# FelixWaiblinger/gym-pybullet-adrp

Measured on AMD Instinct MI355X. Metric: env-steps/sec (N parallel drones) at 1/2/4/8 MI355X; % HBM roofline, higher is better.
Workload: dtype f64; 1 GPU; HoverAviary Physics.PYB 240/30 Hz (8 sub-steps), 4096 envs x 1 drone per GPU, RPM actions, auto-reset; envs_per_gpu=4096, global_envs=4096, drones_per_env=1, parallelism=env-sharded dp1

## Files before the change

### gym_pybullet_adrp_amd/csrc/adrp_device.h

```cpp
#pragma once

#include <hip/hip_runtime.h>
#include <stdint.h>

namespace adrp {

__device__ __forceinline__ void store_out(float4* p, float4 v) {
#ifdef ADRP_NT_STORES
    typedef float f4v __attribute__((ext_vector_type(4)));
    const f4v w = {v.x, v.y, v.z, v.w};
    __builtin_nontemporal_store(w, reinterpret_cast<f4v*>(p));
#else
    *p = v;
#endif
}

#ifdef ADRP_RACE_TIMING
__device__ unsigned long long g_race_phase[32];
#define RACE_MARK(var) const uint64_t var = __builtin_amdgcn_s_memtime()
#define RACE_SET(var) var = __builtin_amdgcn_s_memtime()
#define RACE_ACC(i, dt) do { atomicAdd(&g_race_phase[i], (unsigned long long)(dt)); \
        atomicMax(&g_race_phase[10 + (i)], (unsigned long long)(dt)); } while (0)
constexpr int kWaveSlots = 16384;
__device__ unsigned long long g_race_wave[kWaveSlots * 8];
// ... 350 lines not shown

__device__ __forceinline__ float fatan2_(float y, float x) {
    const float ax = fabsf(x), ay = fabsf(y);
    const float mx = fmaxf(ax, ay), mn = fminf(ax, ay);
    const float a = mx > 0.0f ? mn * __builtin_amdgcn_rcpf(mx) : 0.0f;
    const float t = a * a;
    float p = 0.0028487828094512224f;
    p = p * t - 0.016064105555415154f;
    p = p * t + 0.04268398508429527f;
    p = p * t - 0.07503638416528702f;
    p = p * t + 0.10640615969896317f;
    p = p * t - 0.1420356035232544f;
    p = p * t + 0.19992607831954956f;
    p = p * t - 0.3333307206630707f;
    p = p * t + 1.0f;
    float r = a * p;
    if (ay > ax) r = 1.57079632679489661923f - r;
    if (x < 0.0f) r = 3.14159265358979323846f - r;
    return copysignf(r, y);
}
__device__ __forceinline__ double fatan2_(double y, double x) { return f64::atan2(y, x); }
__device__ __forceinline__ float fatan2_nc_(float y, float x) { return fatan2_(y, x); }
__device__ __forceinline__ double fatan2_nc_(double y, double x) { return f64::atan2_nc(y, x); }
__device__ __forceinline__ float fasin_(float s) { return fatan2_(s, __builtin_amdgcn_sqrtf((1.0f - s) * (1.0f + s))); }
__device__ __forceinline__ double fasin_(double s) { return f64::asin(s); }
__device__ __forceinline__ float fexp_(float x) { return __builtin_amdgcn_exp2f(x * 1.4426950408889634f); }
__device__ __forceinline__ double fexp_(double x) { return f64::exp(x); }

template <typename Real>
struct ChainK {
    Real k004, c100, nn_min, near1, tiny;
    Real ts[3], tc[4];
};
template <typename Real>
__device__ __forceinline__ ChainK<Real> chain_consts() {
    return ChainK<Real>{Real(0.04), Real(100), Real(1e-300), Real(1e-9), Real(0.03),
                        {Real(-0.0001984126984126984), Real(0.008333333333333333), Real(-0.16666666666666666)},
                        {Real(2.48015873015873e-05), Real(-0.001388888888888889), Real(0.041666666666666664), Real(-0.5)}};
}
__device__ __forceinline__ void pin(double& x) { asm volatile("" : "+v"(x)); }
__device__ __forceinline__ void pin(float&) {}
template <typename Real>
__device__ __forceinline__ void pin_all(ChainK<Real>& k) {
    pin(k.k004); pin(k.c100); pin(k.nn_min); pin(k.near1); pin(k.tiny);
#pragma unroll
    for (int i = 0; i < 3; ++i) pin(k.ts[i]);
#pragma unroll
    for (int i = 0; i < 4; ++i) pin(k.tc[i]);
}
__device__ __forceinline__ float hsqrt_nn_(float x, const ChainK<float>&) { return __builtin_amdgcn_sqrtf(x); }
__device__ __forceinline__ double hsqrt_nn_(double x, const ChainK<double>& k) {
    const double y = __builtin_amdgcn_rsq(__builtin_fmax(x, k.nn_min));
    double g = x * y, h = 0.5 * y;
#pragma unroll
    for (int i = 0; i < 2; ++i) {
        const double r = f64::fma_(-g, h, 0.5);
        g = f64::fma_(g, r, g);
        h = f64::fma_(h, r, h);
    }
    const double d = f64::fma_(-g, g, x);
    return f64::fma_(d, h, g);
}
__device__ __forceinline__ void expmap_sinc_cos(float x, float* sinc, float* c, const ChainK<float>&) {
    expmap_sinc_cos(x, sinc, c);
}
__device__ __forceinline__ void expmap_sinc_cos(double x, double* sinc, double* c, const ChainK<double>& k) {
    const double x2 = x * x;
    const bool tiny = __builtin_fabs(x) <= k.tiny;
    double ps = f64::fma_(k.ts[0], x2, k.ts[1]);
    ps = f64::fma_(ps, x2, k.ts[2]);
    double pc = f64::fma_(k.tc[0], x2, k.tc[1]);
    pc = f64::fma_(pc, x2, k.tc[2]);
    pc = f64::fma_(pc, x2, k.tc[3]);
    if (__builtin_expect(!__all(tiny), 0)) {
        double fs, fc;
        expmap_sinc_cos_full(x, &fs, &fc);
        *sinc = tiny ? f64::fma_(x2, ps, 1.0) : fs;
        *c = tiny ? f64::fma_(x2, pc, 1.0) : fc;
        return;
    }
    *sinc = f64::fma_(x2, ps, 1.0);
    *c = f64::fma_(x2, pc, 1.0);
}
__device__ __forceinline__ float quat_inv_norm(float n2, const ChainK<float>&) { return quat_inv_norm(n2); }
__device__ __forceinline__ double quat_inv_norm(double n2, const ChainK<double>& k) {
    const bool near1 = __builtin_fabs(n2 - 1.0) <= k.near1;
    const double newton = f64::fma_(0.5, 1.0 - n2, 1.0);
    if (__builtin_expect(__all(near1), 1)) return newton;
    const double r = f64::rsq_nc(n2);
    return near1 ? newton : r;
}

__device__ __forceinline__ void clamp100_wv(V3<float>& w, V3<float>& v) {
    w = {__builtin_amdgcn_fmed3f(w.x, -100.0f, 100.0f), __builtin_amdgcn_fmed3f(w.y, -100.0f, 100.0f),
         __builtin_amdgcn_fmed3f(w.z, -100.0f, 100.0f)};
    v = {__builtin_amdgcn_fmed3f(v.x, -100.0f, 100.0f), __builtin_amdgcn_fmed3f(v.y, -100.0f, 100.0f),
         __builtin_amdgcn_fmed3f(v.z, -100.0f, 100.0f)};
}
__device__ __forceinline__ double clamp100_sel(double x) { return x < -100.0 ? -100.0 : (x > 100.0 ? 100.0 : x); }
__device__ __forceinline__ void clamp100_wv(V3<double>& w, V3<double>& v) {
    const bool big = (__builtin_fabs(w.x) > 100.0) | (__builtin_fabs(w.y) > 100.0) | (__builtin_fabs(w.z) > 100.0) |
                     (__builtin_fabs(v.x) > 100.0) | (__builtin_fabs(v.y) > 100.0) | (__builtin_fabs(v.z) > 100.0);
    if (__builtin_expect(__any(big), 0)) {
        w = {clamp100_sel(w.x), clamp100_sel(w.y), clamp100_sel(w.z)};
        v = {clamp100_sel(v.x), clamp100_sel(v.y), clamp100_sel(v.z)};
    }
}


template <typename Real>
__device__ __forceinline__ M3<Real> rot(Q4<Real> q) {
    const Real x2 = q.x + q.x, y2 = q.y + q.y, z2 = q.z + q.z;
    const Real xx = q.x * x2, yy = q.y * y2, zz = q.z * z2;
    const Real xy = q.x * y2, xz = q.x * z2, yz = q.y * z2;
    const Real wx = q.w * x2, wy = q.w * y2, wz = q.w * z2;
    return {Real(1) - (yy + zz), xy - wz, xz + wy,
            xy + wz, Real(1) - (xx + zz), yz - wx,
            xz - wy, yz + wx, Real(1) - (xx + yy)};
}
template <typename Real>
__device__ __forceinline__ V3<Real> mul(const M3<Real>& R, V3<Real> v) {
    return {R.a00 * v.x + R.a01 * v.y + R.a02 * v.z,
            R.a10 * v.x + R.a11 * v.y + R.a12 * v.z,
            R.a20 * v.x + R.a21 * v.y + R.a22 * v.z};
}
template <typename Real>
__device__ __forceinline__ V3<Real> mulT(const M3<Real>& R, V3<Real> v) {
    return {R.a00 * v.x + R.a10 * v.y + R.a20 * v.z,
            R.a01 * v.x + R.a11 * v.y + R.a21 * v.z,
            R.a02 * v.x + R.a12 * v.y + R.a22 * v.z};
}
template <typename Real>
__device__ __forceinline__ V3<Real> col2(const M3<Real>& R) {
    return {R.a02, R.a12, R.a22};
}

template <typename Real>
__device__ __forceinline__ V3<Real> euler_xyz(Q4<Real> q) {
    const Real sqx = q.x * q.x, sqy = q.y * q.y, sqz = q.z * q.z, squ = q.w * q.w;
    const Real sarg = Real(-2) * (q.x * q.z - q.w * q.y);
    const Real half_pi = Real(1.57079632679489661923);
    if (sarg <= Real(-0.99999)) return {Real(0), -half_pi, Real(2) * atan2_(q.x, -q.y)};
    if (sarg >= Real(0.99999)) return {Real(0), half_pi, Real(2) * atan2_(-q.x, q.y)};
    return {atan2_(Real(2) * (q.y * q.z + q.w * q.x), squ - sqx - sqy + sqz), asin_(sarg),
            atan2_(Real(2) * (q.x * q.y + q.w * q.z), squ + sqx - sqy - sqz)};
}

template <typename Real>
struct EulerArgs {
    Real sarg, y0, x0, y2, x2;
};
template <typename Real>
__device__ __forceinline__ Real euler_sarg(Q4<Real> q) {
#pragma clang fp contract(on)
    return Real(-2) * (q.x * q.z - q.w * q.y);
}
template <typename Real>
__device__ __forceinline__ EulerArgs<Real> euler_args(Q4<Real> q) {
#pragma clang fp contract(on)
    const Real sqx = q.x * q.x, sqy = q.y * q.y, sqz = q.z * q.z, squ = q.w * q.w;
    const Real sarg = Real(-2) * (q.x * q.z - q.w * q.y);
    const Real y0 = Real(2) * (q.y * q.z + q.w * q.x), x0 = squ - sqx - sqy + sqz;
    const Real y2 = Real(2) * (q.x * q.y + q.w * q.z), x2 = squ + sqx - sqy - sqz;
    return {sarg, y0, x0, y2, x2};
}

// ... 115 lines not shown
```

### gym_pybullet_adrp_amd/csrc/hover_kernel.h

```cpp
#pragma once

#include "adrp_device.h"
#include "dslpid_core.h"

namespace adrp {

enum HoverField {
    HF_POS = 0, HF_QUAT = 3, HF_VEL = 7, HF_OMEGA = 10, HF_LAST_RPM = 13, HF_ANGV = 17,
    HF_LINK_QUAT = 20, HF_NBASE = 24,
    HF_PID = 24, HF_NPID = 9
};
enum HoverInt { HI_STEP = 0, HI_EPISODE = 1, HI_RING_HEAD = 2, HI_N = 3 };

template <typename Real>
struct HoverConst {
    int S, trunc_steps, link_lag, physics;
    Real dt, mass, inv_mass, gravity;
    Real ixx, iyy, izz, inv_ixx, inv_iyy, inv_izz;
    Real kf, km, hover_rpm;
    Real px[4], py[4], pz[4];
    Real gnd_kf, prop_r4, gnd_clip;
    Real drag[3];
    Real dyn_arm;
    Real coll_hh, coll_r, coll_zoff;
// ... 279 lines not shown
    const Real ty = (-f[0] + f[1] + f[2] - f[3]) * a.dyn_arm;
    const V3<Real> rr = b.w;
    const V3<Real> tq = v3(tx, ty, tz) - cross(rr, v3(a.ixx * rr.x, a.iyy * rr.y, a.izz * rr.z));
    const V3<Real> rdd = v3(tq.x * a.inv_ixx, tq.y * a.inv_iyy, tq.z * a.inv_izz);
    b.vel = b.vel + a.dt * (a.inv_mass * force_w);
    b.w = rr + a.dt * rdd;
    b.pos = b.pos + a.dt * b.vel;
    const V3<Real> w = b.w;
    const Real wn = hsqrt_(dot(w, w));
    if (!(wn <= Real(1e-8))) {
        const Real th = wn * a.dt * Real(0.5);
        Real s, c;
        if (th <= Real(0.39269908169872414)) small_sincos(th, &s, &c);
        else sincos_(th, &s, &c);
        const Real k = s * rcp_(wn);
        const Q4<Real> q = b.q;
        b.q = {c * q.x + k * (w.z * q.y - w.y * q.z + w.x * q.w),
               c * q.y + k * (-w.z * q.x + w.x * q.z + w.y * q.w),
               c * q.z + k * (w.y * q.x - w.x * q.y + w.z * q.w),
               c * q.w + k * (-w.x * q.x - w.y * q.y - w.z * q.z)};
    }
    b.angv = mul(R, b.w);
}

template <typename Real>
__device__ __forceinline__ void hover_reset_draw(const HoverReset<Real>& a, uint64_t seed, uint64_t gid, uint32_t tag,
                                                 const HoverConst<Real>& C, Body<Real>& b, int32_t& sc, int32_t& ep) {
    const U4 r0 = draw(seed, gid, uint32_t(ep), tag, 0);
    const U4 r1 = draw(seed, gid, uint32_t(ep), tag, 1);
    const U4 r2 = draw(seed, gid, uint32_t(ep), tag, 2);
    const uint32_t w0[4] = {r0.a, r0.b, r0.c, r0.d}, w1[4] = {r1.a, r1.b, r1.c, r1.d},
                   w2[4] = {r2.a, r2.b, r2.c, r2.d};
    Real p[3], e_[3], v[3], om[3];
#pragma unroll
    for (int k = 0; k < 3; ++k) {
        p[k] = a.init_xyz[k] + a.n_xyz[k] * (Real(2) * u01r<Real>(w0[k]) - Real(1));
        e_[k] = a.init_rpy[k] + a.n_rpy[k] * (Real(2) * u01r<Real>(w1[k]) - Real(1));
        v[k] = a.n_vel[k] * (Real(2) * u01r<Real>(w2[k]) - Real(1));
    }
    om[0] = a.n_om[0] * (Real(2) * u01r<Real>(w0[3]) - Real(1));
    om[1] = a.n_om[1] * (Real(2) * u01r<Real>(w1[3]) - Real(1));
    om[2] = a.n_om[2] * (Real(2) * u01r<Real>(w2[3]) - Real(1));
    b.q = quat_from_euler_fast<Real>(e_[0], e_[1], e_[2]);
    b.pos = v3(p[0], p[1], p[2]);
    b.ql = b.q;
    b.vel = v3(v[0], v[1], v[2]);
    if (C.physics == ADRP_PHYS_DYN) {
        b.w = mulT(rot(b.q), v3(om[0], om[1], om[2]));
        b.angv = v3(om[0], om[1], om[2]);
    } else {
        b.w = v3(om[0], om[1], om[2]);
        b.angv = v3(Real(0), Real(0), Real(0));
    }
#pragma unroll
    for (int i = 0; i < 4; ++i) b.prev_rpm[i] = Real(0);
    sc = 0;
    ep += 1;
}
template <typename Real>
__device__ __forceinline__ void hover_reset_state(const HoverArgs<Real>& args, const HoverConst<Real>& C, int e,
                                                  Body<Real>& b, int32_t& sc, int32_t& ep) {
    hover_reset_draw(*args.r, args.seed, uint64_t(args.env_offset + e), TAG_HOVER_RESET, C, b, sc, ep);
}

template <typename Real>
__device__ __forceinline__ Real euler_roll_u(Q4<Real> q) {
    if (__builtin_expect(__any(fabs_(euler_sarg(q)) >= Real(0.99999)), 0)) return euler_xyz_fast(q).x;
    const EulerArgs<Real> a = euler_args(q);
    return fatan2_(a.y0, a.x0);
}
template <typename Real>
__device__ __forceinline__ Real euler_pitch_u(Q4<Real> q) {
    const Real sarg = euler_sarg(q);
    if (__builtin_expect(__any(fabs_(sarg) >= Real(0.99999)), 0)) return euler_xyz_fast(q).y;
    return fasin_(sarg);
}
template <typename Real>
__device__ __forceinline__ Real euler_yaw_u(Q4<Real> q) {
    if (__builtin_expect(__any(fabs_(euler_sarg(q)) >= Real(0.99999)), 0)) return euler_xyz_fast(q).z;
    const EulerArgs<Real> a = euler_args(q);
    return fatan2_(a.y2, a.x2);
}

template <typename Real>
__device__ __forceinline__ Real euler_axis_u(Q4<Real> q, int ax) {
    const EulerArgs<Real> a = euler_args(q);
    const Real sarg = a.sarg;
    if (__builtin_expect(__any(fabs_(sarg) >= Real(0.99999)), 0)) {
        const V3<Real> r = euler_xyz_fast(q);
        return ax == 0 ? r.x : (ax == 1 ? r.y : r.z);
    }
    const Real y0 = a.y0, x0 = a.x0, y2 = a.y2, x2 = a.x2;
    Real x1;
    if constexpr (sizeof(Real) == 8) x1 = f64::sqrt((1.0 - sarg) * (1.0 + sarg));
    else x1 = __builtin_amdgcn_sqrtf((1.0f - sarg) * (1.0f + sarg));
    const Real yy = ax == 0 ? y0 : (ax == 1 ? sarg : y2), xx = ax == 0 ? x0 : (ax == 1 ? x1 : x2);
    return fatan2_(yy, xx);
}
__device__ __forceinline__ float readlane_r(float v, int l) {
    return __int_as_float(__builtin_amdgcn_readlane(__float_as_int(v), l));
}
__device__ __forceinline__ double readlane_r(double v, int l) {
    return __hiloint2double(__builtin_amdgcn_readlane(__double2hiint(v), l), __builtin_amdgcn_readlane(__double2loint(v), l));
}
template <typename Real>
__device__ __forceinline__ V3<Real> hover_obs12_split(const HoverConst<Real>& a, const Body<Real>& b, float o[12]) {
    const int l = int(threadIdx.x) & 63;
    const Real ang = euler_axis_u(b.q, l < 2 ? l : 2);
    const V3<Real> rpy = v3(readlane_r(ang, 0), readlane_r(ang, 1), readlane_r(ang, 2));
    const V3<Real> w = a.physics == ADRP_PHYS_DYN ? b.angv : b.w;
    o[0] = float(b.pos.x); o[1] = float(b.pos.y); o[2] = float(b.pos.z);
    o[3] = float(rpy.x);   o[4] = float(rpy.y);   o[5] = float(rpy.z);
    o[6] = float(b.vel.x); o[7] = float(b.vel.y); o[8] = float(b.vel.z);
    o[9] = float(w.x);     o[10] = float(w.y);    o[11] = float(w.z);
    return rpy;
}

template <typename Real>
__device__ __forceinline__ V3<Real> hover_obs12(const HoverConst<Real>& a, const Body<Real>& b, float o[12]) {
    const V3<Real> rpy = euler_xyz_fast_u(b.q);
    const V3<Real> w = a.physics == ADRP_PHYS_DYN ? b.angv : b.w;
    o[0] = float(b.pos.x); o[1] = float(b.pos.y); o[2] = float(b.pos.z);
    o[3] = float(rpy.x);   o[4] = float(rpy.y);   o[5] = float(rpy.z);
    o[6] = float(b.vel.x); o[7] = float(b.vel.y); o[8] = float(b.vel.z);
    o[9] = float(w.x);     o[10] = float(w.y);    o[11] = float(w.z);
    return rpy;
}

template <int A, int B>
__device__ __forceinline__ void write_row(float* row, const float o12[12], const float (&ring)[B][A], int head1) {
    if constexpr (A == 4) {
        float4* r4 = reinterpret_cast<float4*>(row);
        r4[0] = make_float4(o12[0], o12[1], o12[2], o12[3]);
        r4[1] = make_float4(o12[4], o12[5], o12[6], o12[7]);
        r4[2] = make_float4(o12[8], o12[9], o12[10], o12[11]);
#pragma unroll
        for (int p = 0; p < B; ++p) {
            int k = p - head1;
            k += k < 0 ? B : 0;
            r4[3 + k] = make_float4(ring[p][0], ring[p][1], ring[p][2], ring[p][3]);
        }
    } else {
#pragma unroll
        for (int k = 0; k < 12; ++k) row[k] = o12[k];
#pragma unroll
        for (int p = 0; p < B; ++p) {
            int k = p - head1;
            k += k < 0 ? B : 0;
#pragma unroll
            for (int j = 0; j < A; ++j) row[12 + k * A + j] = ring[p][j];
        }
    }
}

template <int A>
__device__ __forceinline__ void write_row_generic(float* __restrict__ row, const float o12[12],
                                                  const float* __restrict__ ring, int B, int E, int e, int head1,
                                                  const float act[A], bool act_is_newest) {
#pragma unroll
    for (int k = 0; k < 12; ++k) row[k] = o12[k];
    constexpr int CH = 8;
    int slot = head1;
    for (int k0 = 0; k0 < B; k0 += CH) {
        float v[CH][A];
#pragma unroll
        for (int c = 0; c < CH; ++c) {
// ... 207 lines not shown
        const Real r2 = rpm[i] * rpm[i];
        const Real f = r2 * C.kf;
        sum_f += f;
        const bool pz0 = __builtin_constant_p(C.pz[i]) && C.pz[i] == Real(0);
        const Real fx = f * C.px[i], fy = f * C.py[i], fz = f * C.pz[i];
        P = v3(P.x + fx, P.y + fy, pz0 ? P.z : P.z + fz);
        t2 += (i & 1) ? -r2 : r2;
    }
    const Real tau_z = t2 * C.km;
    ChainK<Real> K = chain_consts<Real>();
    HoverConst<Real> Cp = C;
    if constexpr (sizeof(Real) == 8) {
        pin_all(K);
        pin(Cp.dt); pin(Cp.mass); pin(Cp.gravity); pin(Cp.inv_mass); pin(Cp.ang_max);
        pin(Cp.ixx); pin(Cp.iyy); pin(Cp.izz); pin(Cp.inv_ixx); pin(Cp.inv_iyy); pin(Cp.inv_izz);
        pin(Cp.coll_hh); pin(Cp.coll_r); pin(Cp.coll_zoff);
    }
    Chain<Real> st{};
    {
        const M3<Real> R = rot_fm(b.q);
        const M3<Real> Rs = lag ? rot_fm(b.ql) : R;
        st.wb = mulT(R, b.w);
        st.zc = col2(R);
        st.zs = col2(Rs);
        st.m3 = lag ? mulT(R, st.zs) : v3(Real(0), Real(0), Real(1));
        if constexpr (DRAG) {
            st.R = R;
            st.Rs = Rs;
        }
    }
    st.wn = hsqrt_nn_(dot(b.w, b.w), K);
    st.dti = v3(Cp.dt * Cp.inv_ixx, Cp.dt * Cp.inv_iyy, Cp.dt * Cp.inv_izz);
    bool touched = false;
    auto substep = [&](int s) {
        if constexpr (EXT) touched |= pyb_substep<Real, PH, true>(Cp, b, st, rpm, sum_f, P, tau_z, K, ext(b, st));
        else touched |= pyb_substep<Real, PH>(Cp, b, st, rpm, sum_f, P, tau_z, K, V3<Real>{}, vxy ? vxy + 2 * s : nullptr);
#pragma unroll
        for (int i = 0; i < 4; ++i) b.prev_rpm[i] = rpm[i];
    };
    if constexpr (SC > 0) {
#pragma unroll
        for (int s = 0; s < SC; ++s) substep(s);
    } else {
        for (int s = 0; s < C.S; ++s) substep(s);
    }
    if (wb_out) *wb_out = st.wb;
    else b.w = mul(rot_fm(b.q), st.wb);
    return touched;
}

constexpr int kRowF4 = 18;

template <int A, int B>
__device__ __forceinline__ void stage_row(float4* lds_row, const float o12[12], const float (&ring)[B][A], int head1) {
    lds_row[0] = make_float4(o12[0], o12[1], o12[2], o12[3]);
    lds_row[1] = make_float4(o12[4], o12[5], o12[6], o12[7]);
    lds_row[2] = make_float4(o12[8], o12[9], o12[10], o12[11]);
#pragma unroll
    for (int p = 0; p < B; ++p) {
        int k = p - head1;
        k += k < 0 ? B : 0;
        lds_row[3 + k] = make_float4(ring[p][0], ring[p][1], ring[p][2], ring[p][3]);
    }
}

template <typename Real, int PH, int A, int B, int SC, bool STG = false, int CTL = 0, bool HELP = false, int SYS = 0,
          int FO = 2>
__device__ __forceinline__ void hover_step_body(const HoverArgs<Real>& a, const HoverConst<Real>& C,
                                                const float* pre = nullptr) {
    constexpr int BR = B > 0 ? B : 1;
    constexpr bool DRAG = (PH == ADRP_PHYS_PYB_DRAG || PH == ADRP_PHYS_PYB_GND_DRAG_DW);
    constexpr bool DYN = (PH == ADRP_PHYS_DYN);
    static_assert(!HELP || STG, "the reset helper wave pairs with the staged (all lanes live) kernel");
    __shared__ Real rs_body[HELP ? kResetFields * kStepBlock : 1];
    __shared__ float rs_obs[HELP ? 12 * kStepBlock : 1];
    __shared__ float4 rows[STG ? kStepBlock * kRowF4 : 1];
    constexpr bool ANG = HELP && angle_helpers<Real>();
    __shared__ Real ang_q[ANG ? 4 * kStepBlock : 1];
    __shared__ Real ang_r[ANG ? kStepBlock : 1];
    __shared__ Real ang_p[ANG ? kStepBlock : 1];
    __shared__ float ang_y[ANG ? kStepBlock : 1];
    constexpr int kWaves = HELP ? 1 + help_waves<Real>() : 1;
    constexpr auto cb = [](int w) { return w == 0 ? 0 : (w >= kWaves ? kRowF4 : (kWaves == 2 ? kRowF4 / 2 : 5 * w - 2)); };
    if constexpr (HELP) {
        if (ANG && threadIdx.x >= 2 * kStepBlock) {
            const int tl = threadIdx.x & (kStepBlock - 1), wv = threadIdx.x / kStepBlock;
            __syncthreads();
            const Q4<Real> q = {ang_q[tl], ang_q[kStepBlock + tl], ang_q[2 * kStepBlock + tl], ang_q[3 * kStepBlock + tl]};
            if (wv == 2) ang_p[tl] = euler_pitch_u(q);
            else ang_y[tl] = float(euler_yaw_u(q));
            __syncthreads();
            __syncthreads();
            float4* dst = reinterpret_cast<float4*>(a.obs) + size_t(blockIdx.x) * kStepBlock * kRowF4;
            for (int k = cb(wv); k < cb(wv + 1); ++k) store_out(dst + tl + kStepBlock * k, rows[tl + kStepBlock * k]);
            return;
        }
        if (threadIdx.x >= kStepBlock) {
            const int tl = threadIdx.x - kStepBlock;
            const int he = blockIdx.x * kStepBlock + tl;
            const int E = a.E;
            const float4 av = reinterpret_cast<const float4*>(a.act)[he];
            float rg[BR][4];
#pragma unroll
            for (int p = 0; p < B; ++p) {
                const float4 v = reinterpret_cast<const float4*>(a.ring)[size_t(p) * E + he];
                rg[p][0] = v.x; rg[p][1] = v.y; rg[p][2] = v.z; rg[p][3] = v.w;
            }
            const int32_t head = a.ist[HI_RING_HEAD * E + he];
            int32_t hsc = 0, hep = a.ist[HI_EPISODE * E + he];
            Body<Real> rb;
            hover_reset_state(a, C, he, rb, hsc, hep);
            float o[12];
            hover_obs12(C, rb, o);
            const Real v[kResetFields] = {rb.pos.x, rb.pos.y, rb.pos.z, rb.q.x, rb.q.y, rb.q.z, rb.q.w,
                                          rb.vel.x, rb.vel.y, rb.vel.z, rb.w.x, rb.w.y, rb.w.z,
                                          rb.angv.x, rb.angv.y, rb.angv.z};
#pragma unroll
            for (int k = 0; k < kResetFields; ++k) rs_body[k * kStepBlock + tl] = v[k];
#pragma unroll
            for (int k = 0; k < 12; ++k) rs_obs[k * kStepBlock + tl] = o[k];
            float4* my = rows + tl * kRowF4;
            const int hu = __builtin_amdgcn_readfirstlane(head);
            if (__all(head == hu)) {
                const int h1 = hu + 1 == B ? 0 : hu + 1;
#pragma unroll
                for (int p = 0; p < B; ++p) {
                    const int k = p >= h1 ? p - h1 : p - h1 + B;
                    my[3 + k] = make_float4(rg[p][0], rg[p][1], rg[p][2], rg[p][3]);
                }
                my[3 + B - 1] = av;
            } else {
                const int h1 = head + 1 == B ? 0 : head + 1;
#pragma unroll
                for (int p = 0; p < B; ++p) {
                    int k = p - h1;
                    k += k < 0 ? B : 0;
                    const bool hit = p == head;
                    my[3 + k] = make_float4(hit ? av.x : rg[p][0], hit ? av.y : rg[p][1], hit ? av.z : rg[p][2],
                                            hit ? av.w : rg[p][3]);
                }
            }
            reinterpret_cast<float4*>(a.ring)[size_t(head) * E + he] = av;
            __syncthreads();
            if constexpr (ANG) {
                const Q4<Real> q = {ang_q[tl], ang_q[kStepBlock + tl], ang_q[2 * kStepBlock + tl], ang_q[3 * kStepBlock + tl]};
                ang_r[tl] = euler_roll_u(q);
                __syncthreads();
            }
            __syncthreads();
            float4* dst = reinterpret_cast<float4*>(a.obs) + size_t(blockIdx.x) * kStepBlock * kRowF4;
#pragma unroll
            for (int k = cb(1); k < cb(2); ++k) store_out(dst + tl + kStepBlock * k, rows[tl + kStepBlock * k]);
            return;
        }
    }
    const int E = a.E;
    const bool split = ADRP_PERSIST_SPLIT && !STG && !HELP && E == 1;
    const int e = split ? 0 : int(blockIdx.x) * kStepBlock + int(threadIdx.x);
    const int D = B > 0 ? 12 + B * A : a.D;
    if (e >= E) return;
    RACE_MARK(t0);
    const bool fit = FO == 2 ? field_offsets_fit<Real>(E) : FO == 1;
    const bool lag = C.link_lag && !DYN;
    const BodyOffs<Real> fo = body_offsets<Real>(E, e, lag, DRAG, DYN);
    uint32_t io[HI_N];
    field_run(uint32_t(e) * 4u, uint32_t(E) * 4u, 0, HI_N, io);
    Body<Real> b;
    int32_t sc, ep, head_ld;
    if (fit) {
        load_body_at<Real>(a.f, fo, b, lag, DRAG, DYN);
        sc = field_at(a.ist, io[HI_STEP]); ep = field_at(a.ist, io[HI_EPISODE]); head_ld = field_at(a.ist, io[HI_RING_HEAD]);
        field_form_end();
    } else {
        load_body(a, e, b, lag, DRAG, DYN);
        sc = a.ist[HI_STEP * E + e]; ep = a.ist[HI_EPISODE * E + e]; head_ld = a.ist[HI_RING_HEAD * E + e];
    }
    const int32_t head = head_ld;
    float act[A];
    if constexpr (SYS == 2) {
#pragma unroll
        for (int j = 0; j < A; ++j) act[j] = pre[j];
    } else if constexpr (SYS == 1) {
        uint32_t* sa = const_cast<uint32_t*>(reinterpret_cast<const uint32_t*>(a.act)) + size_t(e) * A;
#pragma unroll
        for (int j = 0; j < A; ++j)
            act[j] = __uint_as_float(__hip_atomic_load(sa + j, __ATOMIC_RELAXED, __HIP_MEMORY_SCOPE_SYSTEM));
    } else if constexpr (A == 4) {
        const float4 v = reinterpret_cast<const float4*>(a.act)[e];
        act[0] = v.x; act[1] = v.y; act[2] = v.z; act[3] = v.w;
    } else {
#pragma unroll
        for (int j = 0; j < A; ++j) act[j] = a.act[e * A + j];
    }
    float ring[BR][A];
#pragma unroll
    for (int p = 0; p < (HELP ? 0 : B); ++p) {
        if constexpr (A == 4) {
            const float4 v = reinterpret_cast<const float4*>(a.ring)[size_t(p) * E + e];
            ring[p][0] = v.x; ring[p][1] = v.y; ring[p][2] = v.z; ring[p][3] = v.w;
        } else {
#pragma unroll
            for (int j = 0; j < A; ++j) ring[p][j] = a.ring[(size_t(p) * E + e) * A + j];
        }
    }
    Real rpm[4];
    if constexpr (CTL != 0) {
        static_assert(A == (CTL == ADRP_ACT_PID ? 3 : CTL == ADRP_ACT_VEL ? 4 : 1), "PID action width");
        Real ctl[HF_NPID];
        uint32_t po[HF_PID + HF_NPID];
        field_run(uint32_t(e) * uint32_t(sizeof(Real)), uint32_t(E) * uint32_t(sizeof(Real)), HF_PID, HF_NPID, po);
        if (fit) {
#pragma unroll
            for (int k = 0; k < HF_NPID; ++k) ctl[k] = field_at(a.f, po[HF_PID + k]);
            field_form_end();
        } else {
#pragma unroll
            for (int k = 0; k < HF_NPID; ++k) ctl[k] = a.f[(HF_PID + k) * E + e];
        }
        dslpid_rpm<Real, CTL>(C, b, act, ctl, rpm);
        if (fit) {
#pragma unroll
            for (int k = 0; k < HF_NPID; ++k) field_last(a.f, po[HF_PID + k]) = ctl[k];
            field_form_end();
        } else {
#pragma unroll
            for (int k = 0; k < HF_NPID; ++k) a.f[(HF_PID + k) * E + e] = ctl[k];
        }
    } else {
#pragma unroll
        for (int i = 0; i < 4; ++i) rpm[i] = C.hover_rpm * Real(rpm_gain(act[A == 1 ? 0 : i]));
    }
    bool touched = false;
// ... 42 lines not shown
    V3<Real> rpy;
    if constexpr (ANG) {
        const int tl = threadIdx.x;
        ang_q[tl] = b.q.x; ang_q[kStepBlock + tl] = b.q.y; ang_q[2 * kStepBlock + tl] = b.q.z;
        ang_q[3 * kStepBlock + tl] = b.q.w;
        __syncthreads();
        hold(b.q.x); hold(b.q.y); hold(b.q.z); hold(b.q.w);
        hold(wbf.x); hold(wbf.y); hold(wbf.z);
        hold(b.pos.x); hold(b.pos.y); hold(b.pos.z);
        if constexpr (LATE_XY) {
#pragma unroll
            for (int k = 0; k < 2 * SC; ++k) hold(vxy[k]);
#pragma unroll
            for (int s = 0; s < SC; ++s) {
                b.pos.x = fmx(C.dt, vxy[2 * s], b.pos.x);
                b.pos.y = fmx(C.dt, vxy[2 * s + 1], b.pos.y);
            }
        }
        hold(b.vel.x); hold(b.vel.y); hold(b.vel.z);
        if constexpr (!DYN) b.w = mul(rot_fm(b.q), wbf);
        const V3<Real> w = C.physics == ADRP_PHYS_DYN ? b.angv : b.w;
        o12[0] = float(b.pos.x); o12[1] = float(b.pos.y); o12[2] = float(b.pos.z);
        o12[6] = float(b.vel.x); o12[7] = float(b.vel.y); o12[8] = float(b.vel.z);
        o12[9] = float(w.x);     o12[10] = float(w.y);    o12[11] = float(w.z);
    } else if (split) {
        rpy = hover_obs12_split(C, b, o12);
    } else {
        rpy = hover_obs12(C, b, o12);
    }
    const Real dx = C.target[0] - b.pos.x, dy = C.target[1] - b.pos.y, dz = C.target[2] - b.pos.z;
    const Real d2 = dx * dx + dy * dy + dz * dz;
    const Real r = Real(2) - d2 * d2;
    a.rew[e] = float(r > Real(0) ? r : Real(0));
    const bool te = d2 < Real(1e-8);
    bool tr = fabs_(b.pos.x) > Real(1.5) || fabs_(b.pos.y) > Real(1.5) || b.pos.z > Real(2.0) || sc >= C.trunc_steps;
    if constexpr (ANG) {
        hold(b.w.x); hold(b.w.y); hold(b.w.z);
#pragma unroll
        for (int k = 0; k < 12; ++k)
            if (k < 3 || k > 5) hold(o12[k]);
        __syncthreads();
        rpy.x = ang_r[threadIdx.x];
        rpy.y = ang_p[threadIdx.x];
        o12[3] = float(rpy.x);
        o12[4] = float(rpy.y);
        o12[5] = ang_y[threadIdx.x];
    }
    tr = tr || fabs_(rpy.x) > Real(0.4) || fabs_(rpy.y) > Real(0.4);
    a.term[e] = te;
    a.trunc[e] = tr;
    sc += C.S;
    const bool done = a.autoreset && (te || tr);
    RACE_MARK(t3);
#ifdef ADRP_RACE_TIMING
    const unsigned long long dmask = __ballot(done);
    uint64_t t4 = 0;
#endif
    if constexpr (STG) {
        static_assert(A == 4 && B == 15, "staged rows: 72-float rows only");
        float4* my = rows + threadIdx.x * kRowF4;
        const int hu = __builtin_amdgcn_readfirstlane(head);
        if constexpr (HELP) {
        } else if (__all(head == hu)) {
            const int h1 = hu + 1 == B ? 0 : hu + 1;
#pragma unroll
            for (int p = 0; p < B; ++p) {
                const int k = p >= h1 ? p - h1 : p - h1 + B;
                my[3 + k] = make_float4(ring[p][0], ring[p][1], ring[p][2], ring[p][3]);
            }
            my[3 + B - 1] = make_float4(act[0], act[1], act[2], act[3]);
        } else {
#pragma unroll
            for (int p = 0; p < B; ++p) {
                const bool hit = p == head;
#pragma unroll
                for (int j = 0; j < A; ++j) ring[p][j] = hit ? act[j] : ring[p][j];
            }
            stage_row<A, B>(my, o12, ring, head1);
        }
        my[0] = make_float4(o12[0], o12[1], o12[2], o12[3]);
        my[1] = make_float4(o12[4], o12[5], o12[6], o12[7]);
        my[2] = make_float4(o12[8], o12[9], o12[10], o12[11]);
        if constexpr (HELP && !ANG) __syncthreads();
        if (done) {
            if (a.tobs) {
                float4 t[kRowF4];
#pragma unroll
                for (int k = 0; k < kRowF4; ++k) t[k] = my[k];
                float4* trow = reinterpret_cast<float4*>(a.tobs + size_t(e) * D);
#pragma unroll
                for (int k = 0; k < kRowF4; ++k) trow[k] = t[k];
            }
            if constexpr (HELP) {
                const int t = threadIdx.x;
                Real v[kResetFields];
#pragma unroll
                for (int k = 0; k < kResetFields; ++k) v[k] = rs_body[k * kStepBlock + t];
                b.pos = v3(v[0], v[1], v[2]);
                b.q = {v[3], v[4], v[5], v[6]};
                b.ql = b.q;
                b.vel = v3(v[7], v[8], v[9]);
                b.w = v3(v[10], v[11], v[12]);
                b.angv = v3(v[13], v[14], v[15]);
#pragma unroll
                for (int i = 0; i < 4; ++i) b.prev_rpm[i] = Real(0);
                sc = 0;
                ep += 1;
#pragma unroll
                for (int k = 0; k < 12; ++k) o12[k] = rs_obs[k * kStepBlock + t];
            } else {
                hover_reset_state(a, C, e, b, sc, ep);
                hover_obs12(C, b, o12);
            }
            my[0] = make_float4(o12[0], o12[1], o12[2], o12[3]);
            my[1] = make_float4(o12[4], o12[5], o12[6], o12[7]);
            my[2] = make_float4(o12[8], o12[9], o12[10], o12[11]);
        }
        RACE_SET(t4);
        store_state();
        __syncthreads();
        float4* dst = reinterpret_cast<float4*>(a.obs) + size_t(blockIdx.x) * kStepBlock * kRowF4;
        constexpr int KC = cb(1);
#pragma unroll
        for (int k = 0; k < KC; ++k) store_out(dst + threadIdx.x + kStepBlock * k, rows[threadIdx.x + kStepBlock * k]);
    } else {
#pragma unroll
        for (int p = 0; p < B; ++p) {
            const bool hit = p == head;
#pragma unroll
            for (int j = 0; j < A; ++j) ring[p][j] = hit ? act[j] : ring[p][j];
        }
        if (done) {
            if (a.tobs) {
                if constexpr (B > 0) write_row<A, B>(a.tobs + size_t(e) * D, o12, ring, head1);
                else write_row_generic<A>(a.tobs + size_t(e) * D, o12, a.ring, a.B, E, e, head1, act, true);
            }
            hover_reset_state(a, C, e, b, sc, ep);
            if (split) hover_obs12_split(C, b, o12);
            else hover_obs12(C, b, o12);
        }
        RACE_SET(t4);
        if constexpr (B > 0) write_row<A, B>(a.obs + size_t(e) * D, o12, ring, head1);
        else write_row_generic<A>(a.obs + size_t(e) * D, o12, a.ring, a.B, E, e, head1, act, true);
    }
    RACE_MARK(t5);
    if constexpr (!STG) {
        store_state();
    }
#ifdef ADRP_RACE_TIMING
    RACE_MARK(t6);
    if (threadIdx.x == 0) {
        RACE_ACC(0, t1 - t0); RACE_ACC(1, t2 - t1); RACE_ACC(2, t3 - t2); RACE_ACC(3, t4 - t3);
        RACE_ACC(4, t5 - t4); RACE_ACC(5, t6 - t5); RACE_ACC(6, t6 - t0); RACE_ACC(8, 1);
        RACE_ACC(7, __popcll(dmask));
        if (dmask) atomicAdd(&g_race_phase[9], 1ull);
    }
#endif
}

template <typename Real>
struct HoverTail {
    const HoverConst<Real>* c;
    const HoverReset<Real>* r;
    uint8_t* term;
    uint8_t* trunc;
    float* tobs;
    int32_t* contact_count;
    uint64_t seed;
// ... 44 lines not shown
```

Before: 729.0 million env-steps/s.

## Use lean f64 atan2/asin in helper waves and offload terminal-obs rows to helpers

Replaces the general f64 atan2/asin in the euler roll/pitch/yaw helper waves with a lean polynomial atan2 and a Newton-refined sqrt asin. Both fall back to the old path wave-wide when inputs are near the singularity or badly scaled. It also moves the terminal-observation copy for done envs off the main wave: the main wave writes only the first 3 float4s and records a ballot-ranked list of done lanes in shared memory, and the helper waves copy the remaining columns alongside their normal obs stores. The aim is to shorten the helper critical path and the main wave's scattered tobs writes, at the cost of more shared-memory bookkeeping and a tail loop over the done rows.

```diff
diff --git a/gym_pybullet_adrp_amd/csrc/adrp_device.h b/gym_pybullet_adrp_amd/csrc/adrp_device.h
--- a/gym_pybullet_adrp_amd/csrc/adrp_device.h
+++ b/gym_pybullet_adrp_amd/csrc/adrp_device.h
@@ -456,6 +456,62 @@
     *sinc = f64::fma_(x2, ps, 1.0);
     *c = f64::fma_(x2, pc, 1.0);
 }
+struct AngK {
+    double p[10];
+    double tan8, pi4, pi2, pi;
+    double lim, lo, hi;
+};
+__device__ __forceinline__ AngK ang_consts() {
+    return AngK{{0.021428368220326288, -0.04375458729368037, 0.05699267039194693, -0.06642647883966969,
+                 0.07690277001250925, -0.09090800003785938, 0.11111107550967636, -0.14285714221246087,
+                 0.19999999999459742, -0.3333333333333199},
+                0.41421356237309504880, 0.78539816339744830962, 1.57079632679489661923, 3.14159265358979323846,
+                0.99999, 1e-150, 1e150};
+}
+__device__ __forceinline__ void pin_all(AngK& k) {
+#pragma unroll
+    for (int i = 0; i < 10; ++i) pin(k.p[i]);
+    pin(k.tan8); pin(k.pi4); pin(k.pi2); pin(k.pi); pin(k.lim); pin(k.lo); pin(k.hi);
+}
+namespace f64 {
+__device__ __forceinline__ bool atan2_lean_ok(double y, double x, const AngK& k) {
+    const double s = __builtin_fabs(x) + __builtin_fabs(y);
+    return s > k.lo && s < k.hi;
+}
+template <bool XPOS>
+__device__ __forceinline__ double atan2_lean(double y, double x, const AngK& k) {
+    const double ax = __builtin_fabs(x), ay = __builtin_fabs(y);
+    const double mx = __builtin_fmax(ax, ay), mn = __builtin_fmin(ax, ay);
+    const bool big = mn > k.tan8 * mx;
+    const double num = big ? mn - mx : mn, den = big ? mn + mx : mx;
+    const double t = num * rcp_nc(den);
+    const double s = t * t;
+    double p = k.p[0];
+#pragma unroll
+    for (int i = 1; i < 10; ++i) p = fma_(p, s, k.p[i]);
+    double r = fma_(t * s, p, t);
+    if (big) r += k.pi4;
+    if (ay > ax) r = k.pi2 - r;
+    if constexpr (!XPOS) {
+        if (x < 0.0) r = k.pi - r;
+    }
+    return __builtin_copysign(r, y);
+}
+__device__ __forceinline__ double asin_lean(double s, const AngK& k) {
+    const double x = (1.0 - s) * (1.0 + s);
+    const double y = __builtin_amdgcn_rsq(x);
+    double g = x * y, h = 0.5 * y;
+#pragma unroll
+    for (int i = 0; i < 2; ++i) {
+        const double r = fma_(-g, h, 0.5);
+        g = fma_(g, r, g);
+        h = fma_(h, r, h);
+    }
+    const double d = fma_(-g, g, x);
+    return atan2_lean<true>(s, fma_(d, h, g), k);
+}
+}
+
 __device__ __forceinline__ float quat_inv_norm(float n2, const ChainK<float>&) { return quat_inv_norm(n2); }
 __device__ __forceinline__ double quat_inv_norm(double n2, const ChainK<double>& k) {
     const bool near1 = __builtin_fabs(n2 - 1.0) <= k.near1;
diff --git a/gym_pybullet_adrp_amd/csrc/hover_kernel.h b/gym_pybullet_adrp_amd/csrc/hover_kernel.h
--- a/gym_pybullet_adrp_amd/csrc/hover_kernel.h
+++ b/gym_pybullet_adrp_amd/csrc/hover_kernel.h
@@ -385,6 +385,24 @@
     return fatan2_(a.y2, a.x2);
 }
 
+__device__ __forceinline__ double euler_roll_lean(Q4<double> q, const AngK& k) {
+    const EulerArgs<double> a = euler_args(q);
+    const bool ok = fabs_(a.sarg) < k.lim && f64::atan2_lean_ok(a.y0, a.x0, k);
+    if (__builtin_expect(__any(!ok), 0)) return euler_roll_u(q);
+    return f64::atan2_lean<false>(a.y0, a.x0, k);
+}
+__device__ __forceinline__ double euler_pitch_lean(Q4<double> q, const AngK& k) {
+    const double sarg = euler_sarg(q);
+    if (__builtin_expect(__any(!(fabs_(sarg) < k.lim)), 0)) return euler_pitch_u(q);
+    return f64::asin_lean(sarg, k);
+}
+__device__ __forceinline__ double euler_yaw_lean(Q4<double> q, const AngK& k) {
+    const EulerArgs<double> a = euler_args(q);
+    const bool ok = fabs_(a.sarg) < k.lim && f64::atan2_lean_ok(a.y2, a.x2, k);
+    if (__builtin_expect(__any(!ok), 0)) return euler_yaw_u(q);
+    return f64::atan2_lean<false>(a.y2, a.x2, k);
+}
+
 template <typename Real>
 __device__ __forceinline__ Real euler_axis_u(Q4<Real> q, int ax) {
     const EulerArgs<Real> a = euler_args(q);
@@ -758,15 +776,52 @@
     __shared__ float ang_y[ANG ? kStepBlock : 1];
     constexpr int kWaves = HELP ? 1 + help_waves<Real>() : 1;
     constexpr auto cb = [](int w) { return w == 0 ? 0 : (w >= kWaves ? kRowF4 : (kWaves == 2 ? kRowF4 / 2 : 5 * w - 2)); };
+    constexpr bool TROWS = ANG;
+    constexpr int kSplitCols = 5, kSplitRows = 12;
+    static_assert(!TROWS || (cb(2) - cb(1) == kSplitCols && cb(4) - cb(3) == kSplitCols && cb(1) == 3 &&
+                             kSplitCols * kSplitRows <= kStepBlock), "terminal rows: 3 + 3 x 5 columns");
+    __shared__ int done_cnt[1];
+    __shared__ uint8_t done_list[TROWS ? kStepBlock : 1];
+    [[maybe_unused]] auto helper_tail = [&](int tl, int wv) {
+        const int cnt_v = done_cnt[0];
+        const int sub = tl / kSplitCols, c = cb(wv) + tl - kSplitCols * sub;
+        const int row0 = done_list[sub] & (kStepBlock - 1);
+        float4* dst = reinterpret_cast<float4*>(a.obs) + size_t(blockIdx.x) * kStepBlock * kRowF4;
+        float4 o[kSplitCols];
+#pragma unroll
+        for (int j = 0; j < kSplitCols; ++j) o[j] = rows[tl + kStepBlock * (cb(wv) + j)];
+        const float4 t0 = rows[row0 * kRowF4 + c];
+#pragma unroll
+        for (int j = 0; j < kSplitCols; ++j) store_out(dst + tl + kStepBlock * (cb(wv) + j), o[j]);
+        const int cnt = __builtin_amdgcn_readfirstlane(cnt_v);
+        const bool mine = tl < kSplitCols * kSplitRows;
+        float4* tb = reinterpret_cast<float4*>(a.tobs) + size_t(blockIdx.x) * kStepBlock * kRowF4;
+        if (mine && sub < cnt) tb[row0 * kRowF4 + c] = t0;
+        for (int base = kSplitRows; base < cnt && base < kStepBlock; base += kSplitRows) {
+            const int n = base + sub;
+            if (mine && n < cnt) {
+                const int row = done_list[n] & (kStepBlock - 1);
+                tb[row * kRowF4 + c] = rows[row * kRowF4 + c];
+            }
+        }
+    };
     if constexpr (HELP) {
         if (ANG && threadIdx.x >= 2 * kStepBlock) {
             const int tl = threadIdx.x & (kStepBlock - 1), wv = threadIdx.x / kStepBlock;
+            AngK ak = ang_consts();
+            pin_all(ak);
             __syncthreads();
             const Q4<Real> q = {ang_q[tl], ang_q[kStepBlock + tl], ang_q[2 * kStepBlock + tl], ang_q[3 * kStepBlock + tl]};
-            if (wv == 2) ang_p[tl] = euler_pitch_u(q);
-            else ang_y[tl] = float(euler_yaw_u(q));
+            if constexpr (ANG) {
+                if (wv == 2) ang_p[tl] = euler_pitch_lean(q, ak);
+                else ang_y[tl] = float(euler_yaw_lean(q, ak));
+            }
             __syncthreads();
             __syncthreads();
+            if constexpr (TROWS) {
+                helper_tail(tl, wv);
+                return;
+            }
             float4* dst = reinterpret_cast<float4*>(a.obs) + size_t(blockIdx.x) * kStepBlock * kRowF4;
             for (int k = cb(wv); k < cb(wv + 1); ++k) store_out(dst + tl + kStepBlock * k, rows[tl + kStepBlock * k]);
             return;
@@ -817,13 +872,19 @@
                 }
             }
             reinterpret_cast<float4*>(a.ring)[size_t(head) * E + he] = av;
+            [[maybe_unused]] AngK ak = ang_consts();
+            if constexpr (ANG) pin_all(ak);
             __syncthreads();
             if constexpr (ANG) {
                 const Q4<Real> q = {ang_q[tl], ang_q[kStepBlock + tl], ang_q[2 * kStepBlock + tl], ang_q[3 * kStepBlock + tl]};
-                ang_r[tl] = euler_roll_u(q);
+                ang_r[tl] = euler_roll_lean(q, ak);
                 __syncthreads();
             }
             __syncthreads();
+            if constexpr (TROWS) {
+                helper_tail(tl, 1);
+                return;
+            }
             float4* dst = reinterpret_cast<float4*>(a.obs) + size_t(blockIdx.x) * kStepBlock * kRowF4;
 #pragma unroll
             for (int k = cb(1); k < cb(2); ++k) store_out(dst + tl + kStepBlock * k, rows[tl + kStepBlock * k]);
@@ -1032,8 +1093,20 @@
         my[1] = make_float4(o12[4], o12[5], o12[6], o12[7]);
         my[2] = make_float4(o12[8], o12[9], o12[10], o12[11]);
         if constexpr (HELP && !ANG) __syncthreads();
+        if constexpr (TROWS) {
+            const unsigned long long done_mask = __ballot(done);
+            done_cnt[0] = a.tobs ? __popcll(done_mask) : 0;
+            if (done && a.tobs) {
+                float4* trow = reinterpret_cast<float4*>(a.tobs + size_t(e) * D);
+                trow[0] = make_float4(o12[0], o12[1], o12[2], o12[3]);
+                trow[1] = make_float4(o12[4], o12[5], o12[6], o12[7]);
+                trow[2] = make_float4(o12[8], o12[9], o12[10], o12[11]);
+                const uint32_t rank = __builtin_amdgcn_mbcnt_hi(uint32_t(done_mask >> 32), __builtin_amdgcn_mbcnt_lo(uint32_t(done_mask), 0u));
+                done_list[rank] = uint8_t(threadIdx.x);
+            }
+        }
         if (done) {
-            if (a.tobs) {
+            if (!TROWS && a.tobs) {
                 float4 t[kRowF4];
 #pragma unroll
                 for (int k = 0; k < kRowF4; ++k) t[k] = my[k];
```

New measurement: 765.7 million env-steps/s (median of 6 runs). 1.05x the previous value.
